# youthHan/HVRNet

Measured on AMD Instinct MI355X. Metric: VID frames/sec, R101 Faster-RCNN+HVR, 1000x600, 300 props, T=15, higher is better.
Workload: dtype bf16; 1 GPU; configs[2]: faster_rcnn_r101_hrnmp_c5 inference, clip mode; frames_per_window=15, proposals_per_frame=300, input=3x600x1000 padded to 608x1008, parallelism=dp1 independent clips, no collectives, windows_in_flight=4, clips_per_graph=1, key_frame_detections=300

## Files before the change

### hvrnet_amd/csrc/check_regs.py

```python
import os
import re
import sys

SERIAL = 'a serial sweep, scratch traffic inside its dependency chain is a silent slowdown'

RULES = [
    (r'_ZN3hvr17expand_res_kernel', 0, 'expand.hip: sized for two workgroups per CU, a spill means it no longer fits'),
    (r'_ZN3hvr19expand_split_kernel', 0, 'expand_split.hip: sized for two workgroups per CU, a spill means it no longer fits'),
    (r'_ZN3hvr19mc_nms_', 0, 'nms.hip, the per-class read-out and its merge: ' + SERIAL),
    (r'_ZN3hvr15nms_', 0, 'nms.hip, the sort and the mask kernels: ' + SERIAL),
    (r'_ZN3hvr16nms_', 0, 'nms.hip, the greedy sweep with its prefetched IoU rows: ' + SERIAL),
    (r'_ZN3hvr17rpn_', 0, 'nms.hip, the proposal gather / select: ' + SERIAL),
    (r'_ZN3hvr25relation_scores_bt', 0, 'relation_bt.hip: the one-round scores kernel keeps 176 accumulators per lane'),
    (r'_ZN3hvr14pc_tile_kernelI(?:t|NS_5f16_tE)Li4ELi0E', 32,
     'pc_gemm.hip <4, LINEAR, 3>: the fattest compute waves park a few epilogue addresses before the loop'),
    (r'_ZN3hvr14pc_tile_kernelI(?:t|NS_5f16_tE)Li2ELi2E', 256,
     'pc_gemm.hip <2, APPLY, 4>: the folded accumulators are parked between the last block and the epilogue\'s LDS staging'),
    (r'_ZN3hvr14pc_tile_kernel', 0, 'pc_gemm.hip, every other shape: a big accumulator tile, scratch would land in the K loop'),
    (r'_ZN3hvr15big_tile_kernel', 0, 'bigtile.hip: a big accumulator tile, scratch would land in the K loop'),
    (r'_ZN3hvr\d+tta_', 0, 'tta.hip, the augmentation merge: ' + SERIAL),
    (r'_ZN3hvr\d+soft_nms_', 0, 'softnms.hip, the Soft-NMS rounds: ' + SERIAL),
    (r'_ZN3hvr\d+seq_nms_', 0, 'seqnms.hip, the Seq-NMS frame sweep: ' + SERIAL),
    (r'_ZN3hvr\d+deform_im2col_', 0, 'dcn.hip: the sampler keeps four corner vectors in flight per lane'),
    (r'_ZN3hvr\d+deform_roi_pool_', 0, 'dpool.hip: a row of samples, 4 x sample_per_part corner vectors, in flight per lane'),
    (r'_ZN3hvr\d+roi_pool_fwd_', 0, 'roi_pool.hip: a lane keeps the running maxima and indices of its 16-byte piece and the unrolled '
     'walk\'s loads in registers, a spill would sit inside the walk over a bin\'s pixels'),
    (r'_ZN3hvr\d+gconv3x3_', 0, 'gconv3x3.hip: a wave\'s weights stay in registers for its whole life, a spill would put them behind '
     'every tile\'s loads'),
    (r'_ZN3hvr\d+res2_conv3x3_', 0, 'res2.hip: a wave keeps two units\' accumulators and the loads of a whole tap in flight, a spill '
     'would sit inside the K loop'),
    (r'_ZN3hvr\d+gcb_pool_', 0, 'gcb.hip: a wave keeps acc[C / 64] and two pixels\' pieces in registers for its whole run, a spill '
     'would sit on the one pass over the map'),
    (r'_ZN3hvr\d+gn_stats_', 0, 'gn.hip: a lane keeps the running partials of its pieces and two steps\' loads in registers for its '
     'whole run, a spill would sit on the one pass over the map'),
    (r'_ZN3hvr\d+gn_apply_', 0, 'gn.hip: the apply keeps its channels\' mean, scale and shift in registers, a spill would sit on the '
     'one pass over the map'),
    (r'_ZN3hvr\d+gen_attn_', 0, 'gen_attn.hip: a wave keeps its queries, 16 scores and the d / 16 output accumulators in registers '
     'across the key loop, a spill would sit between the two MFMA chains'),
    (r'_ZN3hvr\d+focal_(?:elem|fused)_', 0, 'focal.hip: a lane keeps one 16-byte piece of logits and its results across three library '
     'calls per element, a spill would sit on the one pass over the logits'),
    (r'_ZN3hvr\d+(?:reg_elem|box_pair)_', 0, 'reg_loss.hip: a lane keeps 16-byte pieces of pred, target and weight and the four gradients of a box '
     'pair in registers, a spill would sit on the one pass over the inputs'),
    (r'_ZN3hvr\d+ghm_(?:hist|loss)_', 0, 'ghm.hip: two passes over the elements with a library call each, a spill would sit on the pass'),
]

TILE_KERNEL = r'_ZN3hvr11tile_kernelI(?:t|f|NS_5f16_tE|NS_6f16s_tE)Li(\d+)ELi(\d+)ELi(\d+)ELi(\d+)ELi(\d+)ELb([01])ELb([01])ELi(\d+)E'


def tile_has_untracked_loads(name):
    m = re.match(TILE_KERNEL, name)
    if not m:
        return False
    wm, wn, fm, fn, epi, glds, respre, ns = [int(x) for x in m.groups()]
    bn = wn * fn * 16
    split_pipe = 'f16s_t' in name and ns > 2 and not (wm == 3 and fn == 8)
    return epi == 2 or (ns > 2 and respre == 1 and bn != 256) or split_pipe


def rule_for(name):
    for i, (pattern, allow, _) in enumerate(RULES):
        if re.match(pattern, name):
            return i, allow
    if tile_has_untracked_loads(name):
        return len(RULES), None
    return None


def main(*paths):
    bad, hits, per_unit = [], [0] * (len(RULES) + 1), []
    for p in paths:
        unit, seen = os.path.basename(p).split('.')[0], 0
        blocks = re.split(r'remark: (?:\S+ )?Function Name: ', open(p).read())[1:]
        for b in blocks:
            name = b.split()[0]
            rule = rule_for(name)
            if rule is None:
                continue
            seen += 1
            hits[rule[0]] += 1
            spill = int(re.search(r'VGPRs Spill: (\d+)', b).group(1))
            scratch = int(re.search(r'ScratchSize \[bytes/lane\]: (\d+)', b).group(1))
            allow = rule[1]
            if allow is None:
                if spill:
                    bad.append('%s: %d VGPRs spilled' % (name, spill))
            elif scratch > allow or (spill and not allow):
                bad.append('%s: %d VGPRs spilled, %d bytes of scratch' % (name, spill, scratch))
        per_unit.append((unit, seen, len(blocks)))
    if not sum(hits):
        sys.exit('check_regs: no kernel recognised in the remarks (format change?)')
    stale = [(RULES[i][0] if i < len(RULES) else TILE_KERNEL) for i, n in enumerate(hits) if not n]
    if stale:
        sys.exit('check_regs: these rules match no kernel of the build (stale):\n  ' + '\n  '.join(stale))
    if bad:
        sys.exit('check_regs: these kernels must not spill:\n  ' + '\n  '.join(bad))
    print('check_regs: kernels gated per unit: ' + ', '.join('%s %d of %d' % u for u in per_unit))
    print('check_regs: no rule gates any kernel of: ' + (' '.join(u for u, seen, _ in per_unit if not seen) or '(none)'))
    print('check_regs: %d kernels checked (untracked loads / serial sweeps / big accumulator tiles), none spills' % sum(hits))


if __name__ == '__main__':
    main(*sys.argv[1:])
```

### hvrnet_amd/csrc/expand.hip

```cpp
#include <cstdlib>
#include "common.h"
#include "gemm_params.h"

namespace hvr {

namespace {

__device__ __forceinline__ uint32_t x_lds_off(const void* p) {
  return (uint32_t)(uintptr_t)(const __attribute__((address_space(3))) char*)p;
}
template <int OFF> __device__ __forceinline__ uint4 x_lds_read128(uint32_t addr) {
  static_assert(OFF >= 0 && OFF < 65536, "ds_read offset field");
  uint4 v;
  asm volatile("ds_read_b128 %0, %1 offset:%2" : "=v"(v) : "v"(addr), "n"(OFF));
  return v;
}
template <int N> __device__ __forceinline__ void x_wait_vm() {
  static_assert(N >= 0 && N < 64, "vmcnt is 6 bits");
  __builtin_amdgcn_s_waitcnt((N & 15) | (7 << 4) | (15 << 8) | ((N >> 4) << 14));
}

typedef uint32_t xu32x4 __attribute__((ext_vector_type(4)));

template <int OFF> __device__ __forceinline__ void x_masked_store128(char* dst, const xu32x4& v, uint64_t mask) {
  uint64_t save;
  asm volatile("s_mov_b64 %0, exec\n\ts_and_b64 exec, exec, %1\n\tglobal_store_dwordx4 %2, %3, off offset:%4\n\ts_mov_b64 exec, %0"
               : "=&s"(save) : "s"(mask), "v"(dst), "v"(v), "n"(OFF) : "memory", "scc");
}

constexpr int X_FJ = 4, X_BN = 16 * X_FJ, X_BM = 128, X_NT = 256;

__device__ __forceinline__ int swz_key(int row) { return (((row >> 4) & 3) << 1) | ((row >> 1) & 1); }
__device__ __forceinline__ int nswz_key(int row) { return (((row >> 5) & 1) * 6) | ((row >> 1) & 1); }

}

template <typename HT, int KF, bool RES, int NC, int RF, int NX, bool LIVE = false>
__global__ __launch_bounds__(64 * (X_BM / 16 / RF), RF == 2 ? 2 : 1) void expand_res_kernel(const GemmParams p) {
  constexpr int K = KF * 32, FJ = X_FJ, BN = X_BN, BM = X_BM, NT = 64 * (X_BM / 16 / RF);
  constexpr int CHUNK = BN * K * 2;
  constexpr int SLOTS = CHUNK / 16 / NT;
  static_assert(KF % 2 == 0 && CHUNK % (16 * NT) == 0, "shape");
  constexpr int NV = FJ / 2;
  constexpr int CN = NX * 16, NCHUNK = CN * 128;
  constexpr int NSLOTS = NX > 0 ? NCHUNK / 16 / NT : 0;
  static_assert(NX == 0 || (NX % 4 == 0 && NCHUNK % (16 * NT) == 0), "next-conv shape");
  constexpr int NRES = RES ? RF * NV : 0, NST = RF * NV;
  extern __shared__ __attribute__((aligned(16))) char smem[];

  const int tid = threadIdx.x, lane = tid & 63;
  const int wave = __builtin_amdgcn_readfirstlane(tid >> 6);
  const int q = lane & 15, g = lane >> 4;
  const int m0 = blockIdx.x * BM + wave * 16 * RF;
  const int cb = blockIdx.y * NC;

  auto dma_chunk = [&](int c, char* buf) {
#ifdef HVR_DBG_X_NODMA
    if (c != cb) return;
#endif
#pragma unroll
    for (int i = 0; i < SLOTS; ++i) {
      const int s = i * NT + tid, ks = s / (BN * 8), rem = s - ks * (BN * 8), row = rem >> 3, pos = rem & 7;
      const int ch = pos ^ swz_key(row);
      const char* src = (const char*)p.B + (((long)(c * BN + row) * p.ldb) * 2 + ks * 128 + ch * 16);
      __builtin_amdgcn_global_load_lds((const __attribute__((address_space(1))) void*)src,
                                       (__attribute__((address_space(3))) void*)(buf + (i * NT + wave * 64) * 16), 16, 0, 0);
    }
    if constexpr (NX > 0) {
      char* nbuf = smem + 2 * CHUNK + NC * BN * 4 + (buf == smem ? 0 : NCHUNK);
#pragma unroll
      for (int i = 0; i < NSLOTS; ++i) {
        const int s = i * NT + tid, row = s >> 3, pos = s & 7;
        const int ch = pos ^ nswz_key(row);
        const char* src = (const char*)p.Wn + ((long)row * p.N * 2 + (long)c * 128 + ch * 16);
        __builtin_amdgcn_global_load_lds((const __attribute__((address_space(1))) void*)src,
                                         (__attribute__((address_space(3))) void*)(nbuf + (i * NT + wave * 64) * 16), 16, 0, 0);
      }
    }
  };
  dma_chunk(cb, smem);

  float* shl = reinterpret_cast<float*>(smem + 2 * CHUNK);
  for (int n = tid; n < NC * BN; n += NT) shl[n] = p.bias ? p.bias[cb * BN + n] : 0.f;

  xu32x4 x[RF][KF];
  int mrow[RF], rrow[RF];
  char* crow[LIVE ? RF : 1];
  uint64_t amask[LIVE ? RF : 1];
  static_assert(!LIVE || NX > 0, "the live-store form belongs to the kernels with the next conv");
#pragma unroll
  for (int i = 0; i < RF; ++i) {
    const int m = m0 + i * 16 + q;
    mrow[i] = m < p.M ? m : p.M - 1;
    if constexpr (LIVE) {
      const int ox = mrow[i] % p.OW, t = mrow[i] / p.OW, oy = t % p.OH, b = t / p.OH;
      const int cy = oy / p.live, cx = ox / p.live;
      const bool alive = cy * p.live == oy && cx * p.live == ox;
      const long lrow = ((long)b * ((p.OH - 1) / p.live + 1) + cy) * ((p.OW - 1) / p.live + 1) + cx;
      crow[i] = (char*)p.C + lrow * p.ldc * 2;
      amask[i] = __builtin_amdgcn_ballot_w64(alive);
    }
    rrow[i] = mrow[i];
    if (p.rs > 0) {
      const int ox = mrow[i] % p.OW, t = mrow[i] / p.OW, oy = t % p.OH, b = t / p.OH;
      rrow[i] = (b * p.RH + oy * p.rs) * p.RW + ox * p.rs;
    }
    const char* xr = (const char*)p.A + (long)mrow[i] * p.lda * 2 + g * 16;
    const char* x2r = xr;
    const int kf1 = p.s2 > 0 ? p.K1 / 32 : KF;
    if (p.s2 > 0) {
      const int ox = mrow[i] % p.OW, t = mrow[i] / p.OW, oy = t % p.OH, b = t / p.OH;
      x2r = (const char*)p.A2 + (((long)b * p.H2 + oy * p.s2) * p.W2 + ox * p.s2) * (long)(K - p.K1) * 2 + g * 16;
    }
#pragma unroll
    for (int kf = 0; kf < KF; ++kf)
      x[i][kf] = *reinterpret_cast<const xu32x4*>(kf < kf1 ? xr + kf * 64 : x2r + (kf - kf1) * 64);
  }

  constexpr int RD = 3, AHEAD = RD - 1;
  xu32x4 res[RD][RF][NV];
  auto load_res = [&](int c, xu32x4 (&r)[RF][NV]) {
#ifdef HVR_DBG_X_NORES
    if constexpr (false) {
#else
    if constexpr (RES) {
#endif
#pragma unroll
      for (int i = 0; i < RF; ++i) {
        const char* rr = (const char*)p.resid + ((long)rrow[i] * p.ldr + c * BN + g * 4 * FJ) * 2;
#pragma unroll
        for (int v = 0; v < NV; ++v) r[i][v] = *reinterpret_cast<const xu32x4*>(rr + v * 16);
      }
    }
  };
  __syncthreads();
  load_res(cb, res[0]);
  if constexpr (AHEAD > 1 && NC > 1) load_res(cb + 1, res[1]);

  const int key = ((q >> 2) << 1) | ((q >> 1) & 1);
  const uint32_t w_lane = x_lds_off(smem) + ((q >> 2) * 4 * FJ + (q & 3)) * 128 + ((g ^ key) << 4);
  const uint32_t sh_lane = x_lds_off(shl) + g * 4 * FJ * 4;

  f32x4 hacc[NX > 0 ? RF : 1][NX > 0 ? NX : 1];
  if constexpr (NX > 0) {
#pragma unroll
    for (int i = 0; i < RF; ++i)
#pragma unroll
      for (int j = 0; j < NX; ++j) hacc[i][j] = f32x4{0.f, 0.f, 0.f, 0.f};
  }
  const uint32_t n_lane = x_lds_off(smem) + 2 * CHUNK + NC * BN * 4 + ((q >> 2) * 16 + (q & 3)) * 128;
  const int nkey = ((q >> 3) * 6) | ((q >> 1) & 1);

  static_for<NC>([&](auto U) {
    constexpr int u = decltype(U)::value;
    const int c = cb + u;
    xu32x4 (&rcur)[RF][NV] = res[u % RD];
#if defined(HVR_DBG_X_NORES) || defined(HVR_DBG_X_NOSTORE)
    constexpr int behind = 0;
#else
    constexpr int behind = (AHEAD > 1 && u + 1 < NC ? NRES : 0) + (u > 0 ? NST : 0);
#endif
    x_wait_vm<behind>();
    __builtin_amdgcn_s_barrier();
    __builtin_amdgcn_sched_barrier(0);
    if constexpr (u + 1 < NC) dma_chunk(c + 1, smem + ((u + 1) & 1) * CHUNK);
    if constexpr (u + AHEAD < NC) load_res(c + AHEAD, res[(u + AHEAD) % RD]);
    __builtin_amdgcn_sched_barrier(0);
    const uint32_t base0 = w_lane + (uint32_t)(u & 1) * CHUNK, base1 = base0 ^ 64u;
    const int nb = c * BN + g * 4 * FJ;
    f32x4 acc[RF][FJ];
    constexpr int H = FJ / 2;
    uint4 wf[2][H];
    auto read_half = [&](auto T, auto HF) {
      constexpr int t = decltype(T)::value, hf = decltype(HF)::value;
      static_for<H>([&](auto J) {
        constexpr int j = decltype(J)::value;
        wf[hf][j] = x_lds_read128<(t >> 1) * (BN * 128) + (hf * H + j) * 4 * 128>((t & 1) ? base1 : base0);
      });
    };
    read_half(std::integral_constant<int, 0>{}, std::integral_constant<int, 0>{});
    read_half(std::integral_constant<int, 0>{}, std::integral_constant<int, 1>{});
    static_for<KF>([&](auto T) {
      constexpr int t = decltype(T)::value;
      static_for<2>([&](auto HF) {
        constexpr int hf = decltype(HF)::value;
#ifdef HVR_DBG_X_NOLDS
        asm volatile("s_waitcnt lgkmcnt(0)" ::: "memory");
#else
        if constexpr (t + 1 < KF || hf == 0) asm volatile("s_waitcnt lgkmcnt(%0)" ::"n"(H) : "memory");
        else asm volatile("s_waitcnt lgkmcnt(0)" ::: "memory");
#endif
        __builtin_amdgcn_sched_barrier(0);
#pragma unroll
        for (int j = 0; j < H; ++j)
#pragma unroll
          for (int i = 0; i < RF; ++i) {
            const f32x4 cin = t == 0 ? f32x4{0.f, 0.f, 0.f, 0.f} : acc[i][hf * H + j];
#ifdef HVR_DBG_X_NOMMA
            if (t == 0) acc[i][hf * H + j] = __builtin_bit_cast(f32x4, wf[hf][j]); else acc[i][hf * H + j][0] += __uint_as_float(wf[hf][j].x ^ x[i][t][0]);
#else
            acc[i][hf * H + j] = mfma_half<HT>(wf[hf][j], __builtin_bit_cast(uint4, x[i][t]), cin);
#endif
          }
        __builtin_amdgcn_sched_barrier(0);
#ifdef HVR_DBG_X_NOLDS
        if constexpr (false) read_half(std::integral_constant<int, t + 1>{}, HF);
#else
        if constexpr (t + 1 < KF) read_half(std::integral_constant<int, t + 1>{}, HF);
#endif
        __builtin_amdgcn_sched_barrier(0);
      });
    });
    uint4 yv[NX > 0 ? RF : 1][NV];
    uint4 sh[FJ];
#pragma unroll
    for (int j = 0; j < FJ; ++j) sh[j] = x_lds_read128<0>(sh_lane + (u * BN + 4 * j) * 4);
    asm volatile("s_waitcnt lgkmcnt(0)" ::: "memory");
    __builtin_amdgcn_sched_barrier(0);
#pragma unroll
    for (int i = 0; i < RF; ++i) {
      char* dst;
      if constexpr (LIVE) dst = crow[i] + nb * 2;
      else dst = (char*)p.C + ((long)mrow[i] * p.ldc + nb) * 2;
#pragma unroll
      for (int v = 0; v < NV; ++v) {
        uint32_t o[4];
#pragma unroll
        for (int h = 0; h < 4; ++h) {
          const int j = 2 * v + (h >> 1), r = 2 * (h & 1);
          const uint32_t shw[4] = {sh[j].x, sh[j].y, sh[j].z, sh[j].w};
          float lo = acc[i][j][r] + __uint_as_float(shw[r]);
          float hi = acc[i][j][r + 1] + __uint_as_float(shw[r + 1]);
          if constexpr (RES) {
            float rl, rh;
            unpack2<HT>(rcur[i][v][h], rl, rh);
            lo += rl;
            hi += rh;
          }
          if (p.relu) { lo = fmaxf(lo, 0.f); hi = fmaxf(hi, 0.f); }
          o[h] = pack2<HT>(lo, hi);
        }
#ifdef HVR_DBG_X_NOSTORE
        if (o[0] == 0x12345678u && o[3] == 0x9abcdef0u)
#endif
        if constexpr (LIVE) {
          if (v == 0) x_masked_store128<0>(dst, xu32x4{o[0], o[1], o[2], o[3]}, amask[i]);
          else x_masked_store128<16>(dst, xu32x4{o[0], o[1], o[2], o[3]}, amask[i]);
        } else
        *reinterpret_cast<uint4*>(dst + v * 16) = make_uint4(o[0], o[1], o[2], o[3]);
        if constexpr (NX > 0) yv[i][v] = make_uint4(o[0], o[1], o[2], o[3]);
      }
    }
    __builtin_amdgcn_sched_barrier(0);
    if constexpr (NX > 0) {
      const uint32_t nb0 = n_lane + (uint32_t)(u & 1) * NCHUNK;
      constexpr int ND = NX < 4 ? NX : 4;
      uint4 wq[ND][2];
      auto nread = [&](auto JO) {
        constexpr int jo = decltype(JO)::value;
        constexpr int roff = (64 * (jo >> 2) + 4 * (jo & 3)) * 128;
        wq[jo % ND][0] = x_lds_read128<roff>(nb0 + ((((g << 1) | 0) ^ nkey) << 4));
        wq[jo % ND][1] = x_lds_read128<roff>(nb0 + ((((g << 1) | 1) ^ nkey) << 4));
      };
      static_for<ND>([&](auto JO) { nread(JO); });
      static_for<NX>([&](auto JO) {
        constexpr int jo = decltype(JO)::value;
        constexpr int ahead = (NX - 1 - jo) < (ND - 1) ? (NX - 1 - jo) : (ND - 1);
        asm volatile("s_waitcnt lgkmcnt(%0)" ::"n"(2 * ahead) : "memory");
        __builtin_amdgcn_sched_barrier(0);
#pragma unroll
        for (int i = 0; i < RF; ++i) {
          hacc[i][jo] = mfma_half<HT>(wq[jo % ND][0], __builtin_bit_cast(uint4, yv[i][0]), hacc[i][jo]);
          hacc[i][jo] = mfma_half<HT>(wq[jo % ND][1], __builtin_bit_cast(uint4, yv[i][1]), hacc[i][jo]);
        }
        __builtin_amdgcn_sched_barrier(0);
        if constexpr (jo + ND < NX) nread(std::integral_constant<int, jo + ND>{});
      });
      __builtin_amdgcn_sched_barrier(0);
    }
  });
  if constexpr (NX > 0) {
#pragma unroll
    for (int i = 0; i < RF; ++i) {
      char* dst = (char*)p.Hn + ((long)mrow[i] * CN + g * 16) * 2;
#pragma unroll
      for (int hg = 0; hg < NX / 4; ++hg) {
        const float* bn = p.bias_n + hg * 64 + g * 16;
#pragma unroll
        for (int v = 0; v < 2; ++v) {
          uint32_t o[4];
#pragma unroll
          for (int h = 0; h < 4; ++h) {
            const int j = 2 * v + (h >> 1), r = 2 * (h & 1);
            const float lo = fmaxf(hacc[i][4 * hg + j][r] + bn[4 * j + r], 0.f);
            const float hi = fmaxf(hacc[i][4 * hg + j][r + 1] + bn[4 * j + r + 1], 0.f);
            o[h] = pack2<HT>(lo, hi);
          }
          *reinterpret_cast<uint4*>(dst + hg * 128 + v * 16) = make_uint4(o[0], o[1], o[2], o[3]);
        }
      }
    }
  }
}

static int expand_nc(int M, int N) {
  const int panels = (M + X_BM - 1) / X_BM, nchunks = N / X_BN;
  if (nchunks % 8 == 0 && (long)panels * (nchunks / 8) >= 512) return 8;
  if (nchunks % 4 == 0 && (long)panels * (nchunks / 4) >= 256) return 4;
  if (nchunks % 2 == 0) return 2;
  return 0;
}

bool expand_supported(const GemmParams& p) {
  if ((p.dtype != DT_BF16 && p.dtype != DT_F16) || p.conv || p.out_f32 || p.ksplit_steps > 0) return false;
  if (!(p.K == 64 || p.K == 128 || p.K == 256 || p.K == 512 || (p.K == 384 && p.s2 > 0))) return false;
  if (p.s2 > 0 && (p.K1 % 32 || p.K1 <= 0 || p.K1 >= p.K || (p.K - p.K1) % 8 || (reinterpret_cast<uintptr_t>(p.A2) & 15) || p.resid)) return false;
  if (p.rs < 0 || (p.rs > 0 && (!p.resid || p.OH <= 0 || p.OW <= 0 || p.M % (p.OH * p.OW) || (long)(p.OH - 1) * p.rs >= p.RH ||
                                (long)(p.OW - 1) * p.rs >= p.RW || (long)(p.M / (p.OH * p.OW)) * p.RH * p.RW > 0x7fffffffL))) return false;
  if (p.N % X_BN || p.M < X_BM || expand_nc(p.M, p.N) == 0) return false;
  if (p.lda % 8 || p.ldb % 8 || p.ldc % 8 || (p.resid && p.ldr % 8)) return false;
  const uintptr_t al = reinterpret_cast<uintptr_t>(p.A) | reinterpret_cast<uintptr_t>(p.B) | reinterpret_cast<uintptr_t>(p.C) |
                       reinterpret_cast<uintptr_t>(p.resid);
  if (al & 15) return false;
  if ((long)p.N * p.ldb * 2 >= (1L << 31)) return false;
  return true;
}

template <typename T, int KF, bool RES, int NC, int NX = 0, bool LIVE = false>
static hipError_t launch_expand_nc(const GemmParams& p, hipStream_t stream) {
  constexpr int RF = (KF > 8 || NX >= 16) ? 1 : 2;
  constexpr int lds = 2 * X_BN * KF * 32 * 2 + NC * X_BN * 4 + 2 * NX * 16 * 128;
  static_assert(lds <= (RF == 2 ? 80 : 160) * 1024, "two workgroups per CU (one with 8 waves at K = 512)");
  auto kern = expand_res_kernel<T, KF, RES, NC, RF, NX, LIVE>;
  static std::atomic<unsigned> attr_set_dev{0};
  per_device_once(attr_set_dev, [&] {
    (void)hipFuncSetAttribute(reinterpret_cast<const void*>(kern), hipFuncAttributeMaxDynamicSharedMemorySize, lds);
  });
  hipLaunchKernelGGL(kern, dim3((p.M + X_BM - 1) / X_BM, p.N / X_BN / NC), dim3(64 * (X_BM / 16 / RF)), lds, stream, p);
  return hipGetLastError();
}

template <typename T, int KF, bool RES>
static hipError_t launch_expand_res(const GemmParams& p, hipStream_t stream) {
  switch (expand_nc(p.M, p.N)) {
    case 16:
      if constexpr (KF == 8) return launch_expand_nc<T, KF, RES, 16>(p, stream);
      else return hipErrorInvalidValue;
    case 8: return launch_expand_nc<T, KF, RES, 8>(p, stream);
    case 4: return launch_expand_nc<T, KF, RES, 4>(p, stream);
    case 2: return launch_expand_nc<T, KF, RES, 2>(p, stream);
    default: return hipErrorInvalidValue;
  }
}

template <typename T, int KF>
static hipError_t launch_expand(const GemmParams& p, hipStream_t stream) {
  return p.resid ? launch_expand_res<T, KF, true>(p, stream) : launch_expand_res<T, KF, false>(p, stream);
}

template <typename T>
static hipError_t run_expand_next(const GemmParams& p, hipStream_t stream) {
  if (p.live > 0) {
    if (p.N == 256 && p.Cn == 64 && p.K == 64 && p.resid) return launch_expand_nc<T, 2, true, 4, 4, true>(p, stream);
    if (p.N == 512 && p.Cn == 128 && p.K == 128 && p.resid) return launch_expand_nc<T, 4, true, 8, 8, true>(p, stream);
    return hipErrorInvalidValue;
  }
  if (p.N == 256 && p.Cn == 64) {
    if (p.K == 64 && p.resid) return launch_expand_nc<T, 2, true, 4, 4>(p, stream);
    if (p.K == 128 && !p.resid) return launch_expand_nc<T, 4, false, 4, 4>(p, stream);
  }
  if (p.N == 512 && p.Cn == 128) {
    if (p.K == 128 && p.resid) return launch_expand_nc<T, 4, true, 8, 8>(p, stream);
    if (p.K == 384 && !p.resid) return launch_expand_nc<T, 12, false, 8, 8>(p, stream);
  }
  if (p.N == 1024 && p.Cn == 256 && p.K == 256 && p.resid) return launch_expand_nc<T, 8, true, 16, 16>(p, stream);
  return hipErrorInvalidValue;
}

bool expand_next_supported(const GemmParams& p) {
  if (!p.Wn || !p.Hn || !p.bias_n || !expand_supported(p)) return false;
  if ((reinterpret_cast<uintptr_t>(p.Wn) | reinterpret_cast<uintptr_t>(p.Hn) | reinterpret_cast<uintptr_t>(p.bias_n)) & 15) return false;
  if (p.N == 256 && p.Cn == 64) return (p.K == 64 && p.resid) || (p.K == 128 && !p.resid && p.s2 > 0);
  if (p.N == 512 && p.Cn == 128) return (p.K == 128 && p.resid) || (p.K == 384 && !p.resid && p.s2 > 0);
  if (p.N == 1024 && p.Cn == 256) return p.K == 256 && p.resid && p.s2 == 0 && p.M >= 512 * X_BM;
  return false;
}

bool expand_next_live_supported(const GemmParams& p) {
  if (p.live <= 0 || p.rs != 0 || p.s2 != 0 || !p.resid) return false;
  if (p.OH <= 0 || p.OW <= 0 || p.M % (p.OH * p.OW)) return false;
  if (!expand_next_supported(p)) return false;
  return (p.N == 256 && p.Cn == 64 && p.K == 64) || (p.N == 512 && p.Cn == 128 && p.K == 128);
}

template <typename T>
static hipError_t run_expand_t(const GemmParams& p, hipStream_t stream) {
  if (p.Wn) return run_expand_next<T>(p, stream);
  switch (p.K) {
    case 64: return launch_expand<T, 2>(p, stream);
    case 128: return launch_expand<T, 4>(p, stream);
    case 256: return launch_expand<T, 8>(p, stream);
    case 384: return launch_expand<T, 12>(p, stream);
    case 512: return launch_expand<T, 16>(p, stream);
    default: return hipErrorInvalidValue;
  }
}

hipError_t run_expand(const GemmParams& p, hipStream_t stream) {
  return p.dtype == DT_F16 ? run_expand_t<f16_t>(p, stream) : run_expand_t<bf16_t>(p, stream);
}

}
```

Measured before the change: 182.4 frames/s.

## Split layer-3 expand+next-reduce into producer/consumer wave roles with staged LDS handoff

Adds a warp-specialized kernel for the 1024-channel layer-3 expand fused with the next block's 1x1 reduce. Four waves compute the expand GEMM with bias, residual and ReLU, write the output, and stage it in LDS. The other four waves consume the previous chunk with the next-layer weights, so the two GEMMs run as a pipeline inside one workgroup that uses the whole LDS. In exchange the CU holds only one workgroup, there is a barrier per chunk, and the register budget grows, which brings a new spill gate and a changed RF rule for the old path.

```diff
diff --git a/hvrnet_amd/csrc/check_regs.py b/hvrnet_amd/csrc/check_regs.py
--- a/hvrnet_amd/csrc/check_regs.py
+++ b/hvrnet_amd/csrc/check_regs.py
@@ -6,6 +6,8 @@
 
 RULES = [
     (r'_ZN3hvr17expand_res_kernel', 0, 'expand.hip: sized for two workgroups per CU, a spill means it no longer fits'),
+    (r'_ZN3hvr25expand_next_staged_kernel', 0, 'expand.hip, the stage-split layer-3 tail: two waves per SIMD of up to 256 registers, a spill '
+     'would sit in the chunk loop of either role'),
     (r'_ZN3hvr19expand_split_kernel', 0, 'expand_split.hip: sized for two workgroups per CU, a spill means it no longer fits'),
     (r'_ZN3hvr19mc_nms_', 0, 'nms.hip, the per-class read-out and its merge: ' + SERIAL),
     (r'_ZN3hvr15nms_', 0, 'nms.hip, the sort and the mask kernels: ' + SERIAL),
diff --git a/hvrnet_amd/csrc/expand.hip b/hvrnet_amd/csrc/expand.hip
--- a/hvrnet_amd/csrc/expand.hip
+++ b/hvrnet_amd/csrc/expand.hip
@@ -21,6 +21,15 @@
 }
 
 typedef uint32_t xu32x4 __attribute__((ext_vector_type(4)));
+template <int OFF> __device__ __forceinline__ xu32x4 x_global_load128(const void* ptr) {
+  xu32x4 v;
+  asm volatile("global_load_dwordx4 %0, %1, off offset:%2" : "=v"(v) : "v"(ptr), "n"(OFF) : "memory");
+  return v;
+}
+template <int OFF> __device__ __forceinline__ void x_lds_write128(uint32_t addr, const xu32x4& v) {
+  static_assert(OFF >= 0 && OFF < 65536, "ds_write offset field");
+  asm volatile("ds_write_b128 %0, %1 offset:%2" ::"v"(addr), "v"(v), "n"(OFF) : "memory");
+}
 
 template <int OFF> __device__ __forceinline__ void x_masked_store128(char* dst, const xu32x4& v, uint64_t mask) {
   uint64_t save;
@@ -266,15 +275,26 @@
       static_for<NX>([&](auto JO) {
         constexpr int jo = decltype(JO)::value;
         constexpr int ahead = (NX - 1 - jo) < (ND - 1) ? (NX - 1 - jo) : (ND - 1);
+#ifdef HVR_DBG_X_NOLDS
+        asm volatile("s_waitcnt lgkmcnt(0)" ::: "memory");
+#else
         asm volatile("s_waitcnt lgkmcnt(%0)" ::"n"(2 * ahead) : "memory");
+#endif
         __builtin_amdgcn_sched_barrier(0);
 #pragma unroll
         for (int i = 0; i < RF; ++i) {
+#ifdef HVR_DBG_X_NOMMA
+          hacc[i][jo][0] += __uint_as_float(wq[jo % ND][0].x ^ yv[i][0].x);
+          hacc[i][jo][1] += __uint_as_float(wq[jo % ND][1].x ^ yv[i][1].x);
+#else
           hacc[i][jo] = mfma_half<HT>(wq[jo % ND][0], __builtin_bit_cast(uint4, yv[i][0]), hacc[i][jo]);
           hacc[i][jo] = mfma_half<HT>(wq[jo % ND][1], __builtin_bit_cast(uint4, yv[i][1]), hacc[i][jo]);
+#endif
         }
         __builtin_amdgcn_sched_barrier(0);
+#ifndef HVR_DBG_X_NOLDS
         if constexpr (jo + ND < NX) nread(std::integral_constant<int, jo + ND>{});
+#endif
       });
       __builtin_amdgcn_sched_barrier(0);
     }
@@ -283,6 +303,246 @@
 #pragma unroll
     for (int i = 0; i < RF; ++i) {
       char* dst = (char*)p.Hn + ((long)mrow[i] * CN + g * 16) * 2;
+#pragma unroll
+      for (int hg = 0; hg < NX / 4; ++hg) {
+        const float* bn = p.bias_n + hg * 64 + g * 16;
+#pragma unroll
+        for (int v = 0; v < 2; ++v) {
+          uint32_t o[4];
+#pragma unroll
+          for (int h = 0; h < 4; ++h) {
+            const int j = 2 * v + (h >> 1), r = 2 * (h & 1);
+            const float lo = fmaxf(hacc[i][4 * hg + j][r] + bn[4 * j + r], 0.f);
+            const float hi = fmaxf(hacc[i][4 * hg + j][r + 1] + bn[4 * j + r + 1], 0.f);
+            o[h] = pack2<HT>(lo, hi);
+          }
+          *reinterpret_cast<uint4*>(dst + hg * 128 + v * 16) = make_uint4(o[0], o[1], o[2], o[3]);
+        }
+      }
+    }
+  }
+}
+
+template <typename HT>
+__global__ __launch_bounds__(512, 1) void expand_next_staged_kernel(const GemmParams p) {
+  constexpr int KF = 8, K = 256, FJ = X_FJ, BN = X_BN, BM = X_BM, NT = 512, NC = 16, NX = 16, RF = 2, NV = FJ / 2;
+  constexpr int CHUNK = BN * K * 2, NCHUNK = NX * 16 * 128, YBUF = BM * BN * 2;
+  constexpr int SLOTS = CHUNK / 16 / NT, NSLOTS = NCHUNK / 16 / NT;
+  constexpr int N_OFF = 2 * CHUNK, Y_OFF = 2 * CHUNK + 2 * NCHUNK;
+  constexpr int NRES = RF * NV, NST = RF * NV, NSH = FJ;
+  extern __shared__ __attribute__((aligned(16))) char smem[];
+
+  const int tid = threadIdx.x, lane = tid & 63;
+  const int wave = __builtin_amdgcn_readfirstlane(tid >> 6);
+  const int q = lane & 15, g = lane >> 4;
+  const int pw = wave & 3;
+  const int m0 = blockIdx.x * BM + pw * 16 * RF;
+
+  auto dma_w3 = [&](int c, char* buf) {
+#pragma unroll
+    for (int i = 0; i < SLOTS; ++i) {
+      const int row = tid >> 3, pos = tid & 7;
+      const int ch = pos ^ swz_key(row);
+      const char* src = (const char*)p.B + (((long)(c * BN + row) * p.ldb) * 2 + i * 128 + ch * 16);
+      __builtin_amdgcn_global_load_lds((const __attribute__((address_space(1))) void*)src,
+                                       (__attribute__((address_space(3))) void*)(buf + (i * NT + wave * 64) * 16), 16, 0, 0);
+    }
+  };
+  auto dma_wn = [&](int c, char* nbuf) {
+#pragma unroll
+    for (int i = 0; i < NSLOTS; ++i) {
+      const int s = i * NT + tid, row = s >> 3, pos = s & 7;
+      const int ch = pos ^ nswz_key(row);
+      const char* src = (const char*)p.Wn + ((long)row * p.N * 2 + (long)c * 128 + ch * 16);
+      __builtin_amdgcn_global_load_lds((const __attribute__((address_space(1))) void*)src,
+                                       (__attribute__((address_space(3))) void*)(nbuf + (i * NT + wave * 64) * 16), 16, 0, 0);
+    }
+  };
+  auto dma_step = [&](auto U) {
+    constexpr int u = decltype(U)::value;
+    if constexpr (u + 1 < NC) dma_w3(u + 1, smem + ((u + 1) & 1) * CHUNK);
+    if constexpr (u < NC) dma_wn(u, smem + N_OFF + (u & 1) * NCHUNK);
+  };
+  dma_w3(0, smem);
+
+  int mrow[RF];
+#pragma unroll
+  for (int i = 0; i < RF; ++i) {
+    const int m = m0 + i * 16 + q;
+    mrow[i] = m < p.M ? m : p.M - 1;
+  }
+  const uint32_t y_lane = x_lds_off(smem) + Y_OFF + pw * (RF * NV * 1024) + lane * 16;
+
+  if (wave < 4) {
+    xu32x4 x[RF][KF];
+    int rrow[RF];
+#pragma unroll
+    for (int i = 0; i < RF; ++i) {
+      rrow[i] = mrow[i];
+      if (p.rs > 0) {
+        const int ox = mrow[i] % p.OW, t = mrow[i] / p.OW, oy = t % p.OH, b = t / p.OH;
+        rrow[i] = (b * p.RH + oy * p.rs) * p.RW + ox * p.rs;
+      }
+      const char* xr = (const char*)p.A + (long)mrow[i] * p.lda * 2 + g * 16;
+#pragma unroll
+      for (int kf = 0; kf < KF; ++kf) x[i][kf] = *reinterpret_cast<const xu32x4*>(xr + kf * 64);
+    }
+    constexpr int RD = 3, AHEAD = RD - 1;
+    xu32x4 res[RD][RF][NV];
+    auto load_res = [&](int c, xu32x4 (&r)[RF][NV]) {
+#pragma unroll
+      for (int i = 0; i < RF; ++i) {
+        const char* rr = (const char*)p.resid + ((long)rrow[i] * p.ldr + c * BN + g * 4 * FJ) * 2;
+#pragma unroll
+        for (int v = 0; v < NV; ++v) r[i][v] = *reinterpret_cast<const xu32x4*>(rr + v * 16);
+      }
+    };
+    load_res(0, res[0]);
+    load_res(1, res[1]);
+    const bool has_bias = p.bias != nullptr;
+    const float* sh_base = (has_bias ? p.bias : p.bias_n) + g * 4 * FJ;
+    const int sh_step = has_bias ? BN : 0;
+
+    const int key = ((q >> 2) << 1) | ((q >> 1) & 1);
+    const uint32_t w_lane = x_lds_off(smem) + ((q >> 2) * 4 * FJ + (q & 3)) * 128 + ((g ^ key) << 4);
+
+    static_for<NC + 1>([&](auto U) {
+      constexpr int u = decltype(U)::value;
+      constexpr int behind = (u + 1 < NC ? NRES : 0) + (u > 0 ? NST : 0);
+      asm volatile("s_waitcnt lgkmcnt(0)" ::: "memory");
+      x_wait_vm<behind>();
+      __builtin_amdgcn_s_barrier();
+      __builtin_amdgcn_sched_barrier(0);
+      if constexpr (u < NC) {
+        xu32x4 shv[FJ];
+        const float* shp = sh_base + u * sh_step;
+        shv[0] = x_global_load128<0>(shp);
+        shv[1] = x_global_load128<16>(shp);
+        shv[2] = x_global_load128<32>(shp);
+        shv[3] = x_global_load128<48>(shp);
+        __builtin_amdgcn_sched_barrier(0);
+        dma_step(U);
+        if constexpr (u + AHEAD < NC) load_res(u + AHEAD, res[(u + AHEAD) % RD]);
+        __builtin_amdgcn_sched_barrier(0);
+        xu32x4 (&rcur)[RF][NV] = res[u % RD];
+        const uint32_t base0 = w_lane + (uint32_t)(u & 1) * CHUNK, base1 = base0 ^ 64u;
+        const int nb = u * BN + g * 4 * FJ;
+        f32x4 acc[RF][FJ];
+        constexpr int H = FJ / 2;
+        uint4 wf[2][H];
+        auto read_half = [&](auto T, auto HF) {
+          constexpr int t = decltype(T)::value, hf = decltype(HF)::value;
+          static_for<H>([&](auto J) {
+            constexpr int j = decltype(J)::value;
+            wf[hf][j] = x_lds_read128<(t >> 1) * (BN * 128) + (hf * H + j) * 4 * 128>((t & 1) ? base1 : base0);
+          });
+        };
+        read_half(std::integral_constant<int, 0>{}, std::integral_constant<int, 0>{});
+        read_half(std::integral_constant<int, 0>{}, std::integral_constant<int, 1>{});
+        static_for<KF>([&](auto T) {
+          constexpr int t = decltype(T)::value;
+          static_for<2>([&](auto HF) {
+            constexpr int hf = decltype(HF)::value;
+            if constexpr (t + 1 < KF || hf == 0) asm volatile("s_waitcnt lgkmcnt(%0)" ::"n"(H) : "memory");
+            else asm volatile("s_waitcnt lgkmcnt(0)" ::: "memory");
+            __builtin_amdgcn_sched_barrier(0);
+#pragma unroll
+            for (int j = 0; j < H; ++j)
+#pragma unroll
+              for (int i = 0; i < RF; ++i) {
+                const f32x4 cin = t == 0 ? f32x4{0.f, 0.f, 0.f, 0.f} : acc[i][hf * H + j];
+                acc[i][hf * H + j] = mfma_half<HT>(wf[hf][j], __builtin_bit_cast(uint4, x[i][t]), cin);
+              }
+            __builtin_amdgcn_sched_barrier(0);
+            if constexpr (t + 1 < KF) read_half(std::integral_constant<int, t + 1>{}, HF);
+            __builtin_amdgcn_sched_barrier(0);
+          });
+        });
+        x_wait_vm<(u + 1 < NC ? SLOTS : 0) + NSLOTS + (u + AHEAD < NC ? NRES : 0)>();
+        __builtin_amdgcn_sched_barrier(0);
+        const uint32_t yb = y_lane + (uint32_t)(u & 1) * YBUF;
+#pragma unroll
+        for (int i = 0; i < RF; ++i) {
+          char* dst = (char*)p.C + ((long)mrow[i] * p.ldc + nb) * 2;
+#pragma unroll
+          for (int v = 0; v < NV; ++v) {
+            uint32_t o[4];
+#pragma unroll
+            for (int h = 0; h < 4; ++h) {
+              const int j = 2 * v + (h >> 1), r = 2 * (h & 1);
+              float lo = acc[i][j][r] + (has_bias ? __uint_as_float(shv[j][r]) : 0.f);
+              float hi = acc[i][j][r + 1] + (has_bias ? __uint_as_float(shv[j][r + 1]) : 0.f);
+              float rl, rh;
+              unpack2<HT>(rcur[i][v][h], rl, rh);
+              lo += rl;
+              hi += rh;
+              if (p.relu) { lo = fmaxf(lo, 0.f); hi = fmaxf(hi, 0.f); }
+              o[h] = pack2<HT>(lo, hi);
+            }
+            const xu32x4 ov = {o[0], o[1], o[2], o[3]};
+            *reinterpret_cast<xu32x4*>(dst + v * 16) = ov;
+            if (i == 0 && v == 0) x_lds_write128<0>(yb, ov);
+            else if (i == 0) x_lds_write128<1024>(yb, ov);
+            else if (v == 0) x_lds_write128<2048>(yb, ov);
+            else x_lds_write128<3072>(yb, ov);
+          }
+        }
+        __builtin_amdgcn_sched_barrier(0);
+      }
+    });
+  } else {
+    f32x4 hacc[RF][NX];
+#pragma unroll
+    for (int i = 0; i < RF; ++i)
+#pragma unroll
+      for (int j = 0; j < NX; ++j) hacc[i][j] = f32x4{0.f, 0.f, 0.f, 0.f};
+    const uint32_t n_lane = x_lds_off(smem) + N_OFF + ((q >> 2) * 16 + (q & 3)) * 128;
+    const int nkey = ((q >> 3) * 6) | ((q >> 1) & 1);
+
+    static_for<NC + 1>([&](auto U) {
+      constexpr int u = decltype(U)::value;
+      x_wait_vm<0>();
+      __builtin_amdgcn_s_barrier();
+      __builtin_amdgcn_sched_barrier(0);
+      dma_step(U);
+      __builtin_amdgcn_sched_barrier(0);
+      if constexpr (u > 0) {
+        constexpr int c = u - 1;
+        const uint32_t yb = y_lane + (uint32_t)(c & 1) * YBUF;
+        uint4 yv[RF][NV];
+        yv[0][0] = x_lds_read128<0>(yb);
+        yv[0][1] = x_lds_read128<1024>(yb);
+        yv[1][0] = x_lds_read128<2048>(yb);
+        yv[1][1] = x_lds_read128<3072>(yb);
+        const uint32_t nb0 = n_lane + (uint32_t)(c & 1) * NCHUNK;
+        constexpr int ND = 4;
+        uint4 wq[ND][2];
+        auto nread = [&](auto JO) {
+          constexpr int jo = decltype(JO)::value;
+          constexpr int roff = (64 * (jo >> 2) + 4 * (jo & 3)) * 128;
+          wq[jo % ND][0] = x_lds_read128<roff>(nb0 + ((((g << 1) | 0) ^ nkey) << 4));
+          wq[jo % ND][1] = x_lds_read128<roff>(nb0 + ((((g << 1) | 1) ^ nkey) << 4));
+        };
+        static_for<ND>([&](auto JO) { nread(JO); });
+        static_for<NX>([&](auto JO) {
+          constexpr int jo = decltype(JO)::value;
+          constexpr int ahead = (NX - 1 - jo) < (ND - 1) ? (NX - 1 - jo) : (ND - 1);
+          asm volatile("s_waitcnt lgkmcnt(%0)" ::"n"(2 * ahead) : "memory");
+          __builtin_amdgcn_sched_barrier(0);
+#pragma unroll
+          for (int i = 0; i < RF; ++i) {
+            hacc[i][jo] = mfma_half<HT>(wq[jo % ND][0], yv[i][0], hacc[i][jo]);
+            hacc[i][jo] = mfma_half<HT>(wq[jo % ND][1], yv[i][1], hacc[i][jo]);
+          }
+          __builtin_amdgcn_sched_barrier(0);
+          if constexpr (jo + ND < NX) nread(std::integral_constant<int, jo + ND>{});
+        });
+        __builtin_amdgcn_sched_barrier(0);
+      }
+    });
+#pragma unroll
+    for (int i = 0; i < RF; ++i) {
+      char* dst = (char*)p.Hn + ((long)mrow[i] * (NX * 16) + g * 16) * 2;
 #pragma unroll
       for (int hg = 0; hg < NX / 4; ++hg) {
         const float* bn = p.bias_n + hg * 64 + g * 16;
@@ -328,7 +588,7 @@
 
 template <typename T, int KF, bool RES, int NC, int NX = 0, bool LIVE = false>
 static hipError_t launch_expand_nc(const GemmParams& p, hipStream_t stream) {
-  constexpr int RF = (KF > 8 || NX >= 16) ? 1 : 2;
+  constexpr int RF = KF > 8 ? 1 : 2;
   constexpr int lds = 2 * X_BN * KF * 32 * 2 + NC * X_BN * 4 + 2 * NX * 16 * 128;
   static_assert(lds <= (RF == 2 ? 80 : 160) * 1024, "two workgroups per CU (one with 8 waves at K = 512)");
   auto kern = expand_res_kernel<T, KF, RES, NC, RF, NX, LIVE>;
@@ -359,6 +619,19 @@
 }
 
 template <typename T>
+static hipError_t launch_expand_next_staged(const GemmParams& p, hipStream_t stream) {
+  constexpr int lds = 2 * X_BN * 256 * 2 + 2 * 256 * 128 + 2 * X_BM * X_BN * 2;
+  static_assert(lds == 160 * 1024, "one workgroup per CU, the whole LDS");
+  auto kern = expand_next_staged_kernel<T>;
+  static std::atomic<unsigned> attr_set_dev{0};
+  per_device_once(attr_set_dev, [&] {
+    (void)hipFuncSetAttribute(reinterpret_cast<const void*>(kern), hipFuncAttributeMaxDynamicSharedMemorySize, lds);
+  });
+  hipLaunchKernelGGL(kern, dim3((p.M + X_BM - 1) / X_BM), dim3(512), lds, stream, p);
+  return hipGetLastError();
+}
+
+template <typename T>
 static hipError_t run_expand_next(const GemmParams& p, hipStream_t stream) {
   if (p.live > 0) {
     if (p.N == 256 && p.Cn == 64 && p.K == 64 && p.resid) return launch_expand_nc<T, 2, true, 4, 4, true>(p, stream);
@@ -373,7 +646,7 @@
     if (p.K == 128 && p.resid) return launch_expand_nc<T, 4, true, 8, 8>(p, stream);
     if (p.K == 384 && !p.resid) return launch_expand_nc<T, 12, false, 8, 8>(p, stream);
   }
-  if (p.N == 1024 && p.Cn == 256 && p.K == 256 && p.resid) return launch_expand_nc<T, 8, true, 16, 16>(p, stream);
+  if (p.N == 1024 && p.Cn == 256 && p.K == 256 && p.resid && p.s2 == 0) return launch_expand_next_staged<T>(p, stream);
   return hipErrorInvalidValue;
 }
 
```

Result: no change. 182.3 frames/s (-0.1%).
